# Meryx/ComputeRayTracer

Measured on AMD Instinct MI355X. Metric: Mrays/sec (+ HBM GB/s vs peak), 1080p 250k-tri scene, 1/2/4/8 MI355X, higher is better.
Workload: dtype f32; 1 GPU; S2 atrium250k: 253952 triangles + cornell walls/light, 1920x1080, 64 spp per step (BASELINE config 3)

## Files before the change

computeraytracer_amd/csrc/crt_shade.h:

```cpp
#pragma once
#include "crt_device.h"
#include "crt_math.h"
#include "../../include/crt.h"

namespace crt {

#define CRT_PI 3.14159265359f
#define CRT_INFINITY 2139095040.0f
constexpr uint32_t kMaxDepthPath = 100;
constexpr uint32_t kGrid = 16;
constexpr uint32_t kDiffuse = 0, kLight = 1, kGlass = 2;

struct Rng { uint32_t x, y, z, w; };

__device__ __forceinline__ uint32_t tea(uint32_t v0, uint32_t v1)
{
    uint32_t s0 = 0;
#pragma unroll
    for (int n = 0; n < 16; n++) {
        s0 += 0x9e3779b9u;
        v0 += ((v1 << 4) + 0xa341316cu) ^ (v1 + s0) ^ ((v1 >> 5) + 0xc8013ea4u);
        v1 += ((v0 << 4) + 0xad90777du) ^ (v0 + s0) ^ ((v0 >> 5) + 0x7e95761eu);
    }
    return v0;
// ... 5 lines not shown
    s.y = s.y * 1664525u + 1013904223u;
    s.z = s.z * 1664525u + 1013904223u;
    s.w = s.w * 1664525u + 1013904223u;
    s.x += s.y * s.w; s.y += s.z * s.x; s.z += s.x * s.y; s.w += s.y * s.z;
    s.x ^= s.x >> 16; s.y ^= s.y >> 16; s.z ^= s.z >> 16; s.w ^= s.w >> 16;
    s.x += s.y * s.w; s.y += s.z * s.x; s.z += s.x * s.y; s.w += s.y * s.z;
    return (float)(s.x & 0x00ffffffu) * 5.9604644775390625e-08f;
}

__device__ __forceinline__ f3 xyz(float4 v) { return f3{v.x, v.y, v.z}; }

template <bool LITERAL>
__device__ __forceinline__ bool beats(float t, float t_min, float t_max, uint32_t index,
                                      uint32_t b_index, uint32_t b_slot)
{
    if (LITERAL) return !(t < t_min || t > t_max);
    return (t >= t_min) && (t < t_max || (t == t_max && (b_slot == kNoHit || index > b_index)));
}

template <bool LITERAL>
__device__ __forceinline__ bool hit_test_rec(const float4 A, const float4 B, const float4 C, const float4 D, float hit_pad,
                                             uint32_t slot, f3 o, f3 d, uint32_t exclude, float t_min, float &t_max,
                                             uint32_t &b_index, uint32_t &b_slot)
{
    const uint32_t index = f_bits(B.w);
    if (exclude == index) return false;
    const uint32_t cat = f_bits(A.w) & 3u;
    float t;
    if (cat == 2u) {
        f3 v0 = xyz(A), e1 = xyz(B), e2 = xyz(C);
        f3 pvec = cross(d, e2);
        float det = dot(e1, pvec);
        if (det == 0.0f) return false;
        float inv = 1.0f / det;
        f3 tvec = o - v0;
        float u = dot(tvec, pvec) * inv;
        if (!(u >= 0.0f && u <= 1.0f)) return false;
        f3 qvec = cross(tvec, e1);
        float v = dot(d, qvec) * inv;
        if (!(v >= 0.0f && (u + v) <= 1.0f)) return false;
        t = dot(e2, qvec) * inv;
        if (LITERAL) { if (!(t >= t_min && t <= t_max)) return false; }
        else if (!beats<false>(t, t_min, t_max, index, b_index, b_slot)) return false;
        f3 p = ray_at(o, d, t);
        f3 v1 = v0 + e1, v2 = v0 + e2;
        float pad = hit_pad;
        bool in = p.x >= min_(v0.x, min_(v1.x, v2.x)) - pad && p.x <= max_(v0.x, max_(v1.x, v2.x)) + pad &&
                  p.y >= min_(v0.y, min_(v1.y, v2.y)) - pad && p.y <= max_(v0.y, max_(v1.y, v2.y)) + pad &&
                  p.z >= min_(v0.z, min_(v1.z, v2.z)) - pad && p.z <= max_(v0.z, max_(v1.z, v2.z)) + pad;
        if (!in) return false;
    } else if (cat == 0u) {
        f3 n = xyz(D);
        float ndotd = dot(n, d);
        if (ndotd > 0.0f) { n = -n; ndotd = -ndotd; }
        if (abs_(ndotd) < 0.0001f) return false;
        f3 P0 = xyz(A);
        t = dot(n, P0 - o) / ndotd;
        if (!beats<LITERAL>(t, t_min, t_max, index, b_index, b_slot)) return false;
        f3 m = ray_at(o, d, t) - P0;
        float u = dot(m, xyz(B)) / D.w;
        float v = dot(m, xyz(C)) / C.w;
        if (u < 0.0f || u > 1.0f || v < 0.0f || v > 1.0f) return false;
    } else {
        f3 co = o - xyz(A);
        float a = dot(d, d);
        float b = 2.0f * dot(d, co);
        float c = dot(co, co) - B.y;
        float disc = b * b - 4.0f * a * c;
        if (disc <= 0.0f) return false;
        float sq = sqrt_(disc);
        t = (-b - sq) / (2.0f * a);
        if (LITERAL) {
            if (t < t_min || t > t_max) {
                t = (-b + sq) / (2.0f * a);
                if (t < t_min || t > t_max) return false;
            }
        } else {
            if (t < t_min) t = (-b + sq) / (2.0f * a);
            if (!beats<false>(t, t_min, t_max, index, b_index, b_slot)) return false;
        }
    }
    t_max = t; b_index = index; b_slot = slot;
    return true;
}

template <bool LITERAL>
__device__ __forceinline__ bool hit_test(const DevScene &S, uint32_t slot, f3 o, f3 d, uint32_t exclude,
                                         float t_min, float &t_max, uint32_t &b_index, uint32_t &b_slot)
{
    const float4 A = S.prim[3 * slot + 0];
    const float4 B = S.prim[3 * slot + 1];
    const float4 C = S.prim[3 * slot + 2];
    float4 D = float4{0.0f, 0.0f, 0.0f, 0.0f};
    if (exclude != f_bits(B.w) && (f_bits(A.w) & 3u) == 0u) D = S.primD[slot];
    return hit_test_rec<LITERAL>(A, B, C, D, S.hit_pad, slot, o, d, exclude, t_min, t_max, b_index, b_slot);
}

__device__ __forceinline__ void hit_attributes_rec(const float4 A, const float4 B, const float4 C, const float4 D, f3 o, f3 d,
                                                   float t, f3 &pos, f3 &nrm, uint32_t &meta)
{
    meta = f_bits(A.w);
    const uint32_t cat = meta & 3u;
    pos = ray_at(o, d, t);
    if (cat == 1u) {
        nrm = normalize(pos - xyz(A));
    } else {
        f3 n;
        if (cat == 0u) n = xyz(D);
        else n = normalize(cross(xyz(B), xyz(C)));
        nrm = (dot(n, d) > 0.0f) ? -n : n;
    }
}

__device__ __forceinline__ void hit_attributes(const DevScene &S, uint32_t slot, f3 o, f3 d, float t,
                                               f3 &pos, f3 &nrm, uint32_t &meta)
{
    const float4 A = S.prim[3 * slot + 0];
    const uint32_t cat = f_bits(A.w) & 3u;
    float4 B = float4{0.0f, 0.0f, 0.0f, 0.0f}, C = B, D = B;
    if (cat == 0u) D = S.primD[slot];
    else if (cat == 2u) { B = S.prim[3 * slot + 1]; C = S.prim[3 * slot + 2]; }
    hit_attributes_rec(A, B, C, D, o, d, t, pos, nrm, meta);
}

__device__ __noinline__ void intersect_all(const DevScene &S, f3 o, f3 d, uint32_t exclude, float &t_max,
                                           uint32_t &b_index, uint32_t &b_slot, uint32_t &c_prims)
{
    for (uint32_t i = 0; i < S.nprim; i++)
        hit_test<true>(S, S.slot_of_index[i], o, d, exclude, 0.001f, t_max, b_index, b_slot);
    c_prims += S.nprim;
}

__device__ __forceinline__ bool finite3(f3 v)
{
    return abs_(v.x) < 3.0e38f && abs_(v.y) < 3.0e38f && abs_(v.z) < 3.0e38f;
}

template <bool COUNT>
__device__ __forceinline__ void traverse(const DevScene &S, int *stk, f3 o, f3 d, uint32_t exclude,
                                         bool anyhit, float &t_max, uint32_t &b_index, uint32_t &b_slot,
                                         uint32_t &c_nodes, uint32_t &c_prims)
{
    const float t_min = 0.001f;
    if (S.nprim == 0u) return;
    const float tiny = 1.0e-20f;
    f3 id;
    id.x = 1.0f / (abs_(d.x) > tiny ? d.x : __builtin_copysignf(tiny, d.x));
    id.y = 1.0f / (abs_(d.y) > tiny ? d.y : __builtin_copysignf(tiny, d.y));
    id.z = 1.0f / (abs_(d.z) > tiny ? d.z : __builtin_copysignf(tiny, d.z));
    const f3 oid = f3{o.x * id.x, o.y * id.y, o.z * id.z};
    const uint32_t b_slot_in = b_slot;
    int sp = 0;
    int node = S.root;
    for (;;) {
        if (node >= 0) {
            const float4 *np = S.nodes + 4 * (size_t)node;
            const float4 n0 = np[0], n1 = np[1], n2 = np[2], n3 = np[3];
            float ax = fma_(n0.x, id.x, -oid.x), bx = fma_(n0.w, id.x, -oid.x);
            float ay = fma_(n0.y, id.y, -oid.y), by = fma_(n1.x, id.y, -oid.y);
            float az = fma_(n0.z, id.z, -oid.z), bz = fma_(n1.y, id.z, -oid.z);
            float tn0 = __builtin_fmaxf(__builtin_fmaxf(__builtin_fminf(ax, bx), __builtin_fminf(ay, by)),
                                        __builtin_fmaxf(__builtin_fminf(az, bz), t_min));
            float tf0 = __builtin_fminf(__builtin_fminf(__builtin_fmaxf(ax, bx), __builtin_fmaxf(ay, by)),
                                        __builtin_fminf(__builtin_fmaxf(az, bz), t_max));
            ax = fma_(n1.z, id.x, -oid.x); bx = fma_(n2.y, id.x, -oid.x);
            ay = fma_(n1.w, id.y, -oid.y); by = fma_(n2.z, id.y, -oid.y);
// ... 284 lines not shown
```

computeraytracer_amd/csrc/crt_wavefront.hip:

```cpp
#include "crt_shade.h"
#include "crt_tile_class.h"
#include "crt_launch.h"
#include <algorithm>

namespace crt {

#ifndef CRT_WF_STACK
#define CRT_WF_STACK 32
#endif
#ifndef CRT_WF_REFILL
#define CRT_WF_REFILL 24
#endif
#ifndef CRT_WF_INNER_RUN
#define CRT_WF_INNER_RUN 6
#endif
#ifndef CRT_WF_BURSTS
#define CRT_WF_BURSTS 4
#endif
#ifndef CRT_WF_BVH4
#define CRT_WF_BVH4 1
#endif
#ifndef CRT_WF_LEAF_AT
#define CRT_WF_LEAF_AT 32
#endif
// ... 1239 lines not shown
                        if (k2 < 3.0e38f) { if (sp < kWfStack) stk[sp * 64] = r2; else ovf[(size_t)(sp - kWfStack) * ovl] = r2; sp++; }
                        if (k1 < 3.0e38f) { if (sp < kWfStack) stk[sp * 64] = r1; else ovf[(size_t)(sp - kWfStack) * ovl] = r1; sp++; }
                        if (COUNT) d_max_sp = max(d_max_sp, (uint32_t)sp);
                        node = r0;
                    } else if (sp > 0) {
                        sp--; node = stack_pop(stk, ovf, ovl, sp);
                    } else {
                        node = kNoNode;
                        if (pend == 0) {
                            if (shadow) stnt(&g_vis[slot], (b_slot == b_slot_in) ? 1u : 0u);
                            else stnt(&g_hit[slot], float2{t_max, bits_f(b_slot)});
                            active = false;
                        }
                    }
#else
                    const float4 *np = nodes + 4 * (size_t)node;
                    const float4 n0 = np[0], n1 = np[1], n2 = np[2], n3 = np[3];
                    float ax = fma_(n0.x, id.x, -oid.x), bx = fma_(n0.w, id.x, -oid.x);
                    float ay = fma_(n0.y, id.y, -oid.y), by = fma_(n1.x, id.y, -oid.y);
                    float az = fma_(n0.z, id.z, -oid.z), bz = fma_(n1.y, id.z, -oid.z);
                    float tn0 = __builtin_fmaxf(__builtin_fmaxf(__builtin_fminf(ax, bx), __builtin_fminf(ay, by)),
                                                __builtin_fmaxf(__builtin_fminf(az, bz), t_min));
                    float tf0 = __builtin_fminf(__builtin_fminf(__builtin_fmaxf(ax, bx), __builtin_fmaxf(ay, by)),
                                                __builtin_fminf(__builtin_fmaxf(az, bz), t_max));
                    ax = fma_(n1.z, id.x, -oid.x); bx = fma_(n2.y, id.x, -oid.x);
                    ay = fma_(n1.w, id.y, -oid.y); by = fma_(n2.z, id.y, -oid.y);
                    az = fma_(n2.x, id.z, -oid.z); bz = fma_(n2.w, id.z, -oid.z);
                    float tn1 = __builtin_fmaxf(__builtin_fmaxf(__builtin_fminf(ax, bx), __builtin_fminf(ay, by)),
                                                __builtin_fmaxf(__builtin_fminf(az, bz), t_min));
                    float tf1 = __builtin_fminf(__builtin_fminf(__builtin_fmaxf(ax, bx), __builtin_fmaxf(ay, by)),
                                                __builtin_fminf(__builtin_fmaxf(az, bz), t_max));
                    if (COUNT) c_nodes += 2;
                    const bool h0 = tn0 <= tf0 * 1.0000005f;
                    const bool h1 = tn1 <= tf1 * 1.0000005f;
                    const int r0 = (int)f_bits(n3.x), r1 = (int)f_bits(n3.y);
                    const bool first0 = tn0 <= tn1;
                    if (h0 & h1) {
                        stk[sp * 64] = first0 ? r1 : r0;
                        sp++;
                        node = first0 ? r0 : r1;
                    } else if (h0 | h1) {
                        node = h0 ? r0 : r1;
                    } else if (sp > 0) {
                        sp--; node = stk[sp * 64];
                    } else {
                        node = kNoNode;
                        if (pend == 0) {
                            if (shadow) stnt(&g_vis[slot], (b_slot == b_slot_in) ? 1u : 0u);
                            else stnt(&g_hit[slot], float2{t_max, bits_f(b_slot)});
                            active = false;
                        }
                    }
#endif
                }
            }
        }
    }
    if (COUNT) {
        wave_add(ctl->counters[blockIdx.x % kWfShards] + CRT_CNT_NODES, c_nodes);
        wave_add(ctl->counters[blockIdx.x % kWfShards] + CRT_CNT_PRIMS, c_prims);
        if (lane == 0) {
            atomicAdd(ctl->counters[blockIdx.x % kWfShards] + 8, (unsigned long long)d_inner_it); atomicAdd(ctl->counters[blockIdx.x % kWfShards] + 9, (unsigned long long)d_inner_act);
            atomicAdd(ctl->counters[blockIdx.x % kWfShards] + 10, (unsigned long long)d_leaf_it); atomicAdd(ctl->counters[blockIdx.x % kWfShards] + 11, (unsigned long long)d_leaf_act);
            atomicAdd(ctl->counters[blockIdx.x % kWfShards] + 12, (unsigned long long)d_prim_it); atomicAdd(ctl->counters[blockIdx.x % kWfShards] + 13, (unsigned long long)d_scans); atomicAdd(ctl->counters[blockIdx.x % kWfShards] + 14, (unsigned long long)d_refill);
            atomicAdd(ctl->counters[blockIdx.x % kWfShards] + 15, (unsigned long long)d_refill_lanes);
        }
        for (int off = 32; off > 0; off >>= 1) d_max_sp = max(d_max_sp, (uint32_t)__shfl_xor((int)d_max_sp, off, 64));
        if (lane == 0) atomicMax(&ctl->max_sp[blockIdx.x % kWfShards], d_max_sp);
    }
}

#ifndef CRT_WF_PICK_AT
#define CRT_WF_PICK_AT 8
#endif
#ifndef CRT_WF_PKFMA
#define CRT_WF_PKFMA 0
#endif
#ifndef CRT_WF_LEAF2_AT
#define CRT_WF_LEAF2_AT 28
#endif
#ifndef CRT_WF_STALL_AT
#define CRT_WF_STALL_AT 16
#endif
constexpr int kStk2 = kWfStackLds2;
#ifndef CRT_WF_RING
#define CRT_WF_RING 32
#endif
constexpr uint32_t kRing2 = CRT_WF_RING;

__device__ __forceinline__ int stack_pop2(const int *stk, const int *ovf, size_t ovl, int sp)
{
    int v = stk[(sp < kStk2 ? sp : kStk2 - 1) * 64];
    if (sp >= kStk2) v = *(const volatile int *)(ovf + (size_t)(sp - kStk2) * ovl);
    return v;
}
__device__ __forceinline__ uint32_t mbcnt64(unsigned long long m)
{
    return __builtin_amdgcn_mbcnt_hi((uint32_t)(m >> 32), __builtin_amdgcn_mbcnt_lo((uint32_t)m, 0u));
}
__device__ __forceinline__ unsigned long long hit_key(float t, uint32_t index)
{
    return ((unsigned long long)f_bits(t) << 32) | (unsigned long long)(index == kNoHit ? 0xFFFFFFFFu : 0xFFFFFFFEu - index);
}

#ifndef CRT_WF_T2_WAVES
#define CRT_WF_T2_WAVES 5
#endif
template <bool COUNT>
__global__ __launch_bounds__(64, CRT_WF_T2_WAVES) void k_wf_trace2(const WfParams P, uint32_t it)
{
    __shared__ int lds_stack[kStk2 * 64];
    __shared__ float4 ring[4][kRing2];
    __shared__ uint2 ring_l[kRing2];
    __shared__ unsigned long long cell[64];
    __shared__ uint32_t cslot[64];
    __shared__ uint2 tasks[64];
    WfCtl *ctl = P.ctl;
    const uint4 *__restrict__ nodesq = P.sc.nodes4q;
    const f3 qscale = f3{P.sc.qscale[0], P.sc.qscale[1], P.sc.qscale[2]}, qbase = f3{P.sc.qbase[0], P.sc.qbase[1], P.sc.qbase[2]};
    const float4 *__restrict__ prim = P.sc.prim;
    const float4 *__restrict__ primD = P.sc.primD;
    uint32_t *__restrict__ g_vis = P.vis;
    float2 *__restrict__ g_hit = P.hit;
    const size_t cls_stride = (size_t)P.list_cap * kWfShards;
    const float4 *__restrict__ recA = P.recA + (size_t)((it & 1u) * 4u) * cls_stride;
    const float4 *__restrict__ recB = P.recB + (size_t)((it & 1u) * 4u) * cls_stride;
    const uint4 *__restrict__ recC = P.recC + (size_t)((it & 1u) * 4u) * cls_stride;
    const float hit_pad = P.sc.hit_pad;
    const int root = P.sc.root4;
    int *__restrict__ ovf = P.stack_overflow + ((size_t)blockIdx.x * 64 + lane_id());
    const size_t ovl = P.overflow_lanes;
    const uint32_t nprim = P.sc.nprim;
    const bool fetchD = ((unsigned long long)P.sc.npatch << CRT_WF_PATCH_RECOMPUTE) > (unsigned long long)nprim;
    DevScene S = P.sc;
    S.prim = prim; S.primD = primD;

    const uint32_t ringi = it & 3u;
    const uint32_t lane = lane_id();
    int *stk = lds_stack + lane;
    const float t_min = 0.001f;

    const uint32_t home = wf_home_shard(P);
    uint32_t cur_shard = home, sh_e0 = 0, sh_e1 = 0, sh_e2 = 0, sh_total = 0;
    uint32_t chunk_pos = 0, chunk_end = 0, ring_head = 0, ring_n = 0;
    bool have_shard = false, exhausted = false;
    {
        const WfShard &so = ctl->shard[ringi][cur_shard];
        sh_e0 = so.n[0]; sh_e1 = sh_e0 + so.n[1]; sh_e2 = sh_e1 + so.n[2]; sh_total = sh_e2 + so.n[3];
        have_shard = sh_total > 0u;
    }
    bool active = false;
    int pend = 0;
    f3 o = f3{0, 0, 0}, d = f3{0, 0, 0}, id = f3{0, 0, 0}, oid = f3{0, 0, 0};
    uint32_t excl = 0, slot = 0, b_index = kNoHit, b_slot = kNoHit, b_slot_in = kNoHit;
    float t_max = 0.0f;
    bool shadow = false;
    int node = kNoNode, sp = 0;
    bool gx = false, gy = false, gz = false;
    uint32_t c_nodes = 0, c_prims = 0;
    uint32_t d_inner_it = 0, d_inner_act = 0, d_leaf_it = 0, d_leaf_act = 0, d_prim_it = 0, d_refill = 0, d_refill_lanes = 0, d_scans = 0;
    uint32_t d_max_sp = 0;

    for (;;) {
        const unsigned long long idle = __ballot(!active);
        const int nidle = __popcll(idle);
        if (nidle >= CRT_WF_PICK_AT) {
            if (ring_n == 0u && !exhausted) {
                for (int guard = 0; chunk_pos == chunk_end && !exhausted && guard < 2 * (int)kWfShards; guard++) {
                    if (have_shard) {
                        uint32_t base = 0;
                        if (lane == 0) base = atomicAdd(&ctl->shard[ringi][cur_shard].cur, (uint32_t)kTraceChunk);
                        base = __shfl(base, 0, 64);
                        if (base < sh_total) { chunk_pos = base; chunk_end = min(base + (uint32_t)kTraceChunk, sh_total); break; }
                        have_shard = false;
                    }
                    if (COUNT) d_scans++;
                    const WfShard &sl = ctl->shard[ringi][lane % kWfShards];
                    const uint32_t e0 = sl.n[0], e1 = e0 + sl.n[1], e2 = e1 + sl.n[2], tot = e2 + sl.n[3];
                    const uint32_t cur_l = __hip_atomic_load(&sl.cur, __ATOMIC_RELAXED, __HIP_MEMORY_SCOPE_AGENT);
                    const unsigned long long avail = __ballot(cur_l < tot);
                    if (!avail) { exhausted = true; break; }
                    const uint32_t rot = cur_shard & 63u;
                    const unsigned long long pick = wf_prefer_home(P, avail, home);
                    const unsigned long long rmask = rot ? ((pick >> rot) | (pick << (64u - rot))) : pick;
                    cur_shard = ((uint32_t)(__ffsll((long long)rmask) - 1) + rot) & 63u;
                    sh_e0 = __shfl(e0, (int)cur_shard, 64); sh_e1 = __shfl(e1, (int)cur_shard, 64);
                    sh_e2 = __shfl(e2, (int)cur_shard, 64); sh_total = __shfl(tot, (int)cur_shard, 64);
                    have_shard = true;
                }
                if (chunk_pos < chunk_end) {
                    const uint32_t n = min(kRing2, chunk_end - chunk_pos);
                    bool ok = false;
                    float4 R0 = float4{0, 0, 0, 0}, R1 = R0, R2 = R0, R3 = R0;
                    uint2 RL = uint2{kNoHit, kNoHit};
                    if (lane < n) {
                        const uint32_t idx = chunk_pos + lane;
                        const size_t region = (size_t)cur_shard * P.list_cap;
                        const bool sh = idx >= sh_e1;
                        const size_t g = idx < sh_e0 ? region + idx : idx < sh_e1 ? cls_stride + region + (idx - sh_e0)
                                       : idx < sh_e2 ? 2u * cls_stride + region + (idx - sh_e1) : 3u * cls_stride + region + (idx - sh_e2);
                        const float4 ro = ldnt(&recA[g]), rd = ldnt(&recB[g]);
                        uint4 rc = uint4{0, 0, 0, 0};
                        if (sh) rc = ldnt(&recC[g]);
                        uint32_t r_slot;
                        float r_tmax;
                        ok = true;
                        if (sh) {
                            r_slot = rc.x & kWfListSlot; r_tmax = rd.w;
                            RL = uint2{rc.y, rc.z};
                        } else {
                            r_slot = f_bits(rd.w) & kWfListSlot; r_tmax = CRT_INFINITY;
                            if (f_bits(rd.w) & kWfListAlsoExt) ok = false;
                            else if (nprim == 0u) { g_hit[r_slot] = float2{r_tmax, bits_f(kNoHit)}; ok = false; }
                        }
                        const float tiny = 1.0e-20f;
                        f3 i3;
                        i3.x = 1.0f / (abs_(rd.x) > tiny ? rd.x : __builtin_copysignf(tiny, rd.x));
                        i3.y = 1.0f / (abs_(rd.y) > tiny ? rd.y : __builtin_copysignf(tiny, rd.y));
                        i3.z = 1.0f / (abs_(rd.z) > tiny ? rd.z : __builtin_copysignf(tiny, rd.z));
                        const f3 oi = f3{fma_(qbase.x, i3.x, -(ro.x * i3.x)), fma_(qbase.y, i3.y, -(ro.y * i3.y)), fma_(qbase.z, i3.z, -(ro.z * i3.z))};
                        R0 = ro;
                        R1 = float4{rd.x, rd.y, rd.z, bits_f(r_slot | (sh ? 0x80000000u : 0u))};
                        R2 = float4{qscale.x * i3.x, qscale.y * i3.y, qscale.z * i3.z, r_tmax};
                        R3 = float4{oi.x, oi.y, oi.z, bits_f((i3.x < 0.0f ? 1u : 0u) | (i3.y < 0.0f ? 2u : 0u) | (i3.z < 0.0f ? 4u : 0u))};
                    }
                    const unsigned long long mk = __ballot(ok);
                    if (ok) {
                        const uint32_t e = mbcnt64(mk);
                        ring[0][e] = R0; ring[1][e] = R1; ring[2][e] = R2; ring[3][e] = R3; ring_l[e] = RL;
                    }
                    ring_head = 0; ring_n = (uint32_t)__popcll(mk);
                    chunk_pos += n;
                    if (COUNT) { d_refill++; d_refill_lanes += ring_n; }
                    __builtin_amdgcn_fence(__ATOMIC_RELEASE, "wavefront");
                    __builtin_amdgcn_wave_barrier();
                }
            }
            if (ring_n > 0u) {
                const uint32_t give = min((uint32_t)nidle, ring_n);
                const uint32_t my = mbcnt64(idle);
                if (!active && my < give) {
                    const uint32_t e = ring_head + my;
                    const float4 R0 = ring[0][e], R1 = ring[1][e], R2 = ring[2][e], R3 = ring[3][e];
                    const uint2 RL = ring_l[e];
                    o = xyz(R0); excl = f_bits(R0.w);
                    d = xyz(R1); slot = f_bits(R1.w) & kWfListSlot; shadow = (f_bits(R1.w) >> 31) != 0u;
                    id = xyz(R2); t_max = R2.w;
                    oid = xyz(R3);
                    const uint32_t sg = f_bits(R3.w);
                    gx = (sg & 1u) != 0u; gy = (sg & 2u) != 0u; gz = (sg & 4u) != 0u;
                    b_index = RL.x; b_slot = RL.y; b_slot_in = b_slot;
                    cell[lane] = hit_key(t_max, b_index); cslot[lane] = b_slot;
                    node = root; sp = 0; pend = 0;
                    active = true;
                }
                ring_head += give; ring_n -= give;
            }
        }
        if (__ballot(active) == 0ull) {
            if (exhausted && ring_n == 0u) break;
            continue;
        }

#pragma unroll 1
        for (int pass = 0; pass < 64; pass++) {
            if (active && node < 0 && pend == 0 && sp > 0) {
                pend = node;
                sp--; node = stack_pop2(stk, ovf, ovl, sp);
            }
            const bool inner = active && node >= 0 && node != kNoNode;
            const bool leaf = active && (node < 0 || pend != 0);
            const int ni = __popcll(__ballot(inner)), nl = __popcll(__ballot(leaf)), nb = __popcll(__ballot(active));
            if (nb == 0) break;
            if (pass > 0 && 64 - nb >= CRT_WF_PICK_AT && (ring_n > 0u || !exhausted)) break;
            if (nl >= CRT_WF_LEAF2_AT || ni == 0 || nb - ni >= CRT_WF_STALL_AT) {
                const int lf = pend != 0 ? pend : node;
                const uint32_t cnt = leaf ? ((~(uint32_t)lf) & 7u) + 1u : 0u;
                const unsigned long long c0 = __ballot((cnt & 1u) != 0u), c1 = __ballot((cnt & 2u) != 0u), c2 = __ballot((cnt & 4u) != 0u), c3 = __ballot((cnt & 8u) != 0u);
                const uint32_t pre = mbcnt64(c0) + 2u * mbcnt64(c1) + 4u * mbcnt64(c2) + 8u * mbcnt64(c3);
                const bool incl = leaf && pre + cnt <= 64u;
                const unsigned long long mi = __ballot(incl);
                const uint32_t T = (uint32_t)(__popcll(c0 & mi) + 2 * __popcll(c1 & mi) + 4 * __popcll(c2 & mi) + 8 * __popcll(c3 & mi));
                const uint32_t first = (~(uint32_t)lf) >> 3;
                if (incl) {
                    tasks[pre] = uint2{first, lane};
                    if (cnt > 1u) tasks[pre + 1u] = uint2{first + 1u, lane};
                    if (cnt > 2u) tasks[pre + 2u] = uint2{first + 2u, lane};
                    if (cnt > 3u) tasks[pre + 3u] = uint2{first + 3u, lane};
                    for (uint32_t i = 4; i < cnt; i++) tasks[pre + i] = uint2{first + i, lane};
                }
                __builtin_amdgcn_fence(__ATOMIC_RELEASE, "wavefront");
                __builtin_amdgcn_wave_barrier();
                if (COUNT) { d_leaf_it++; d_leaf_act += T; d_prim_it += 1u; }
                const uint2 tk = lane < T ? tasks[lane] : uint2{0u, lane};
                const int owner = (int)tk.y;
                const uint32_t ps = tk.x;
                float4 A = float4{0, 0, 0, 0}, B = A, C = A, D = A;
                if (lane < T) { A = prim[3 * (size_t)ps + 0]; B = prim[3 * (size_t)ps + 1]; C = prim[3 * (size_t)ps + 2]; if (fetchD) D = primD[ps]; }
                bool from_pend = false;
                if (incl) {
                    from_pend = pend != 0;
                    if (from_pend) pend = 0;
                    else if (sp > 0) { sp--; node = stack_pop2(stk, ovf, ovl, sp); }
                    else node = kNoNode;
                }
                const f3 to = f3{__shfl(o.x, owner, 64), __shfl(o.y, owner, 64), __shfl(o.z, owner, 64)};
                const f3 td = f3{__shfl(d.x, owner, 64), __shfl(d.y, owner, 64), __shfl(d.z, owner, 64)};
                const uint32_t t_excl = (uint32_t)__shfl((int)excl, owner, 64);
                bool acc = false;
                unsigned long long key = 0;
                if (lane < T) {
                    const unsigned long long cur = cell[owner];
                    float tm = bits_f((uint32_t)(cur >> 32));
                    const uint32_t low = (uint32_t)cur;
                    uint32_t bi = low == 0xFFFFFFFFu ? kNoHit : 0xFFFFFFFEu - low;
                    const uint32_t bs0 = low == 0xFFFFFFFFu ? kNoHit : 0xFFFFFFFEu;
                    uint32_t bs = bs0;
                    if ((f_bits(A.w) & 3u) == 2u) tri_test(A, B, C, ps, to, td, t_excl, t_min, hit_pad, tm, bi, bs);
                    else {
                        if (!fetchD && (f_bits(A.w) & 3u) == 0u) { const f3 nn = normalize(cross(xyz(B), xyz(C))); D = float4{nn.x, nn.y, nn.z, dot(xyz(B), xyz(B))}; }
                        hit_test_rec<false>(A, B, C, D, hit_pad, ps, to, td, t_excl, t_min, tm, bi, bs);
                    }
                    if (COUNT && __ballot((f_bits(A.w) & 3u) != 2u) != 0ull) d_scans += 64u;
                    acc = bs != bs0;
                    if (acc) {
                        key = hit_key(tm, bi);
                        atomicMin(&cell[owner], key);
                    }
                    if (COUNT) c_prims++;
                }
                __builtin_amdgcn_fence(__ATOMIC_ACQ_REL, "wavefront");
                __builtin_amdgcn_wave_barrier();
                if (acc && cell[owner] == key) cslot[owner] = ps;
                __builtin_amdgcn_fence(__ATOMIC_ACQ_REL, "wavefront");
                __builtin_amdgcn_wave_barrier();
                if (incl) {
                    const unsigned long long v = cell[lane];
                    const uint32_t low = (uint32_t)v;
                    t_max = bits_f((uint32_t)(v >> 32));
                    b_index = low == 0xFFFFFFFFu ? kNoHit : 0xFFFFFFFEu - low;
                    b_slot = cslot[lane];
                    bool done = false;
                    if (shadow && b_slot != b_slot_in) done = true;
                    else if (node == kNoNode && pend == 0) done = true;
                    if (done) {
                        if (shadow) stnt(&g_vis[slot], (b_slot == b_slot_in) ? 1u : 0u);
                        else stnt(&g_hit[slot], float2{t_max, bits_f(b_slot)});
                        active = false;
                    }
                }
            } else {
                if (COUNT) { d_inner_it++; d_inner_act += (uint32_t)ni; }
                if (inner) {
                    float k0, k1, k2, k3;
                    int r0, r1, r2, r3;
                    const uint4 *nq = (const uint4 *)((const char *)nodesq + ((uint32_t)node << 6));
                    const uint4 Q0 = nq[0], Q1 = nq[1], Q2 = nq[2], Q3 = nq[3];
                    const uint32_t nxa = gx ? Q1.z : Q0.x, nxb = gx ? Q1.w : Q0.y, fxa = gx ? Q0.x : Q1.z, fxb = gx ? Q0.y : Q1.w;
                    const uint32_t nya = gy ? Q2.x : Q0.z, nyb = gy ? Q2.y : Q0.w, fya = gy ? Q0.z : Q2.x, fyb = gy ? Q0.w : Q2.y;
                    const uint32_t nza = gz ? Q2.z : Q1.x, nzb = gz ? Q2.w : Q1.y, fza = gz ? Q1.x : Q2.z, fzb = gz ? Q1.y : Q2.w;
#if CRT_WF_PKFMA
                    {
                        const v2f ix = v2f{id.x, id.x}, iy = v2f{id.y, id.y}, iz = v2f{id.z, id.z};
                        const v2f ox = v2f{oid.x, oid.x}, oy = v2f{oid.y, oid.y}, oz = v2f{oid.z, oid.z};
#define CRT_PK(Q, I, O) __builtin_elementwise_fma(v2f{(float)((Q) & 0xFFFFu), (float)((Q) >> 16)}, I, O)
                        const v2f tnx_a = CRT_PK(nxa, ix, ox), tnx_b = CRT_PK(nxb, ix, ox), tfx_a = CRT_PK(fxa, ix, ox), tfx_b = CRT_PK(fxb, ix, ox);
                        const v2f tny_a = CRT_PK(nya, iy, oy), tny_b = CRT_PK(nyb, iy, oy), tfy_a = CRT_PK(fya, iy, oy), tfy_b = CRT_PK(fyb, iy, oy);
                        const v2f tnz_a = CRT_PK(nza, iz, oz), tnz_b = CRT_PK(nzb, iz, oz), tfz_a = CRT_PK(fza, iz, oz), tfz_b = CRT_PK(fzb, iz, oz);
#undef CRT_PK
#define CRT_QK(K, NX, NY, NZ, FX, FY, FZ) { \
                            const float tn_ = __builtin_fmaxf(__builtin_fmaxf(NX, NY), __builtin_fmaxf(NZ, t_min)); \
                            const float tf_ = __builtin_fminf(__builtin_fminf(FX, FY), __builtin_fminf(FZ, t_max)); \
                            K = (tn_ <= tf_ * 1.0000005f) ? tn_ : 3.0e38f; }
                        CRT_QK(k0, tnx_a.x, tny_a.x, tnz_a.x, tfx_a.x, tfy_a.x, tfz_a.x)
                        CRT_QK(k1, tnx_a.y, tny_a.y, tnz_a.y, tfx_a.y, tfy_a.y, tfz_a.y)
                        CRT_QK(k2, tnx_b.x, tny_b.x, tnz_b.x, tfx_b.x, tfy_b.x, tfz_b.x)
                        CRT_QK(k3, tnx_b.y, tny_b.y, tnz_b.y, tfx_b.y, tfy_b.y, tfz_b.y)
#undef CRT_QK
                    }
#else
#define CRT_QBOX(K, NXQ, NYQ, NZQ, FXQ, FYQ, FZQ) { \
                        const float tn_ = __builtin_fmaxf(__builtin_fmaxf(fma_((float)(NXQ), id.x, oid.x), fma_((float)(NYQ), id.y, oid.y)), \
                                                          __builtin_fmaxf(fma_((float)(NZQ), id.z, oid.z), t_min)); \
                        const float tf_ = __builtin_fminf(__builtin_fminf(fma_((float)(FXQ), id.x, oid.x), fma_((float)(FYQ), id.y, oid.y)), \
                                                          __builtin_fminf(fma_((float)(FZQ), id.z, oid.z), t_max)); \
                        K = (tn_ <= tf_ * 1.0000005f) ? tn_ : 3.0e38f; }
                    CRT_QBOX(k0, nxa & 0xFFFFu, nya & 0xFFFFu, nza & 0xFFFFu, fxa & 0xFFFFu, fya & 0xFFFFu, fza & 0xFFFFu)
                    CRT_QBOX(k1, nxa >> 16, nya >> 16, nza >> 16, fxa >> 16, fya >> 16, fza >> 16)
                    CRT_QBOX(k2, nxb & 0xFFFFu, nyb & 0xFFFFu, nzb & 0xFFFFu, fxb & 0xFFFFu, fyb & 0xFFFFu, fzb & 0xFFFFu)
                    CRT_QBOX(k3, nxb >> 16, nyb >> 16, nzb >> 16, fxb >> 16, fyb >> 16, fzb >> 16)
#undef CRT_QBOX
#endif
                    r0 = (int)Q3.x; r1 = (int)Q3.y; r2 = (int)Q3.z; r3 = (int)Q3.w;
                    if (COUNT) c_nodes += 4;
#define CRT_CAS(ka, ra, kb, rb) { const bool sw_ = kb < ka; const float tk_ = sw_ ? kb : ka; kb = sw_ ? ka : kb; ka = tk_; \
                                  const int tr_ = sw_ ? rb : ra; rb = sw_ ? ra : rb; ra = tr_; }
                    CRT_CAS(k0, r0, k1, r1) CRT_CAS(k2, r2, k3, r3) CRT_CAS(k0, r0, k2, r2) CRT_CAS(k1, r1, k3, r3) CRT_CAS(k1, r1, k2, r2)
#undef CRT_CAS
                    if (k0 < 3.0e38f) {
                        if (k3 < 3.0e38f) { if (sp < kStk2) stk[sp * 64] = r3; else ovf[(size_t)(sp - kStk2) * ovl] = r3; sp++; }
                        if (k2 < 3.0e38f) { if (sp < kStk2) stk[sp * 64] = r2; else ovf[(size_t)(sp - kStk2) * ovl] = r2; sp++; }
                        if (k1 < 3.0e38f) { if (sp < kStk2) stk[sp * 64] = r1; else ovf[(size_t)(sp - kStk2) * ovl] = r1; sp++; }
                        if (COUNT) d_max_sp = max(d_max_sp, (uint32_t)sp);
                        node = r0;
                    } else if (sp > 0) {
                        sp--; node = stack_pop2(stk, ovf, ovl, sp);
                    } else {
                        node = kNoNode;
                        if (pend == 0) {
                            if (shadow) stnt(&g_vis[slot], (b_slot == b_slot_in) ? 1u : 0u);
                            else stnt(&g_hit[slot], float2{t_max, bits_f(b_slot)});
                            active = false;
                        }
                    }
                }
            }
        }
    }
    if (COUNT) {
        wave_add(ctl->counters[blockIdx.x % kWfShards] + CRT_CNT_NODES, c_nodes);
        wave_add(ctl->counters[blockIdx.x % kWfShards] + CRT_CNT_PRIMS, c_prims);
        if (lane == 0) {
            atomicAdd(ctl->counters[blockIdx.x % kWfShards] + 8, (unsigned long long)d_inner_it); atomicAdd(ctl->counters[blockIdx.x % kWfShards] + 9, (unsigned long long)d_inner_act);
            atomicAdd(ctl->counters[blockIdx.x % kWfShards] + 10, (unsigned long long)d_leaf_it); atomicAdd(ctl->counters[blockIdx.x % kWfShards] + 11, (unsigned long long)d_leaf_act);
            atomicAdd(ctl->counters[blockIdx.x % kWfShards] + 12, (unsigned long long)d_prim_it); atomicAdd(ctl->counters[blockIdx.x % kWfShards] + 13, (unsigned long long)d_scans); atomicAdd(ctl->counters[blockIdx.x % kWfShards] + 14, (unsigned long long)d_refill);
            atomicAdd(ctl->counters[blockIdx.x % kWfShards] + 15, (unsigned long long)d_refill_lanes);
        }
        for (int off = 32; off > 0; off >>= 1) d_max_sp = max(d_max_sp, (uint32_t)__shfl_xor((int)d_max_sp, off, 64));
        if (lane == 0) atomicMax(&ctl->max_sp[blockIdx.x % kWfShards], d_max_sp);
    }
}

template <bool COUNT>
__global__ __launch_bounds__(64) void k_wf_finish(const WfParams P, const WfFinishSegs G)
{
    __shared__ int lds_stack[kStackDepth * 64];
    const DevScene &S = P.sc;
    const uint32_t seg = blockIdx.x / G.blocks_per_seg, blk = blockIdx.x % G.blocks_per_seg;
    WfCtl *ctl = G.ctl[seg];
    int *stk = lds_stack + lane_id();
    const uint32_t j = blk * P.tail_bound + threadIdx.x;
    const uint32_t count = min(ctl->side_count[G.batch[seg]], kWfSideCap);
    if (blk == 0 && threadIdx.x == 0 && count > G.blocks_per_seg * P.tail_bound) atomicAdd(&ctl->dropped, count - G.blocks_per_seg * P.tail_bound);
    const bool mine = threadIdx.x < P.tail_bound && j < count;
    const uint32_t slot = G.base[seg] + (mine ? j : 0u);
    uint32_t flags = 0;
    if (mine) flags = P.misc[slot].y;
    bool alive = mine && (flags & kWfAlive);
    bool pend_sh = false, pend_ext = false;
    const bool wide = finish_walks_wide(S);
    ShadeCnt cn;
    uint32_t c_nodes = 0, c_prims = 0;
    for (int guard = 0; guard < 512 && __ballot(alive) != 0ull; guard++) {
        if (alive) {
            const float4 ro = P.ray_o[slot];
            const f3 o = xyz(ro);
            const uint32_t excl = f_bits(ro.w);
            if (pend_sh) {
                const float4 sd = P.sh_d[slot];
                uint32_t how;
                P.vis[slot] = finish_walk_shadow<COUNT>(S, stk, wide, o, xyz(sd), excl, sd.w, P.vis[slot], c_nodes, c_prims, how) ? 1u : 0u;
            }
            if (pend_ext) {
                const float4 rd = P.ray_d[slot];
                if (f_bits(rd.w) == 0u) {
                    float t_max = CRT_INFINITY;
                    uint32_t b_index = kNoHit, b_slot = kNoHit, how;
                    finish_walk_extension<COUNT>(S, stk, wide, o, xyz(rd), excl, t_max, b_index, b_slot, c_nodes, c_prims, how);
                    P.hit[slot] = float2{t_max, bits_f(b_slot)};
                }
            }
            ShadeOut so = shade_body<COUNT, true>(P, slot, true, cn);
            const uint32_t resolved = shade_store<COUNT, true>(P, slot, true, so, cn);
            (void)resolved;
            alive = so.alive; pend_ext = so.emit_ext; pend_sh = so.emit_sh;
        }
    }
    if (alive) atomicAdd(&ctl->dropped, 1u);

    if (COUNT) {
        wave_add(ctl->counters[blockIdx.x % kWfShards] + CRT_CNT_RAYS, cn.rays);
        wave_add(ctl->counters[blockIdx.x % kWfShards] + CRT_CNT_BOUNCES, cn.bounces);
        wave_add(ctl->counters[blockIdx.x % kWfShards] + CRT_CNT_SHADOW, cn.shadow);
        wave_add(ctl->counters[blockIdx.x % kWfShards] + CRT_CNT_HITS, cn.hits);
        wave_add(ctl->counters[blockIdx.x % kWfShards] + CRT_CNT_PATHS, cn.paths);
        wave_add(ctl->counters[blockIdx.x % kWfShards] + CRT_CNT_PRIMS, cn.prims + c_prims);
        wave_add(ctl->counters[blockIdx.x % kWfShards] + CRT_CNT_WALKED, cn.walk);
        wave_add(ctl->counters[blockIdx.x % kWfShards] + CRT_CNT_NODES, c_nodes);
    }
}

__global__ __launch_bounds__(64) void k_wf_resolve(const WfParams P, uint32_t last_sample)
{
    const size_t npix = (size_t)P.tw * P.th;
    const size_t pix = (size_t)blockIdx.x * 64 + threadIdx.x;
// ... 228 lines not shown
```

Before: 8049 Mrays/s.

## Run two inner-node steps per wave iteration when most lanes are inner

Adds an optional double-step of BVH4 inner-node traversal when at least 40 lanes are on inner nodes, so a second node visit happens before returning to the leaf/refill decision loop. Before the second step, a lane holding a leaf with no pending work parks that leaf and pops the next stack entry. Also adds gated-off variants: branch-free flat triangle/patch acceptance tests, and resolving hit slot late from index to drop the cslot LDS array and a barrier. Only the double-step is on by default. It trades extra divergence and longer per-iteration latency for fewer scheduling round trips.

```diff
diff --git a/computeraytracer_amd/csrc/crt_shade.h b/computeraytracer_amd/csrc/crt_shade.h
--- a/computeraytracer_amd/csrc/crt_shade.h
+++ b/computeraytracer_amd/csrc/crt_shade.h
@@ -111,6 +111,52 @@
     }
     t_max = t; b_index = index; b_slot = slot;
     return true;
+}
+
+__device__ __forceinline__ bool beats_flat(float t, float t_min, float t_max, uint32_t index, uint32_t b_index, uint32_t b_slot)
+{
+    return (t >= t_min) & ((t < t_max) | ((t == t_max) & ((b_slot == kNoHit) | (index > b_index))));
+}
+
+__device__ __forceinline__ bool tri_accepts_flat(const float4 A, const float4 B, const float4 C, float hit_pad, f3 o, f3 d,
+                                                 uint32_t exclude, float t_min, float t_max, uint32_t b_index, uint32_t b_slot, float &t)
+{
+    const uint32_t index = f_bits(B.w);
+    const f3 v0 = xyz(A), e1 = xyz(B), e2 = xyz(C);
+    const f3 pvec = cross(d, e2);
+    const float det = dot(e1, pvec);
+    const float inv = 1.0f / det;
+    const f3 tvec = o - v0;
+    const float u = dot(tvec, pvec) * inv;
+    const f3 qvec = cross(tvec, e1);
+    const float v = dot(d, qvec) * inv;
+    t = dot(e2, qvec) * inv;
+    const f3 p = ray_at(o, d, t);
+    const f3 v1 = v0 + e1, v2 = v0 + e2;
+    const f3 lo = f3{min_(v0.x, min_(v1.x, v2.x)) - hit_pad, min_(v0.y, min_(v1.y, v2.y)) - hit_pad, min_(v0.z, min_(v1.z, v2.z)) - hit_pad};
+    const f3 hi = f3{max_(v0.x, max_(v1.x, v2.x)) + hit_pad, max_(v0.y, max_(v1.y, v2.y)) + hit_pad, max_(v0.z, max_(v1.z, v2.z)) + hit_pad};
+    const bool in = (p.x >= lo.x) & (p.x <= hi.x) & (p.y >= lo.y) & (p.y <= hi.y) & (p.z >= lo.z) & (p.z <= hi.z);
+    const bool wins = beats_flat(t, t_min, t_max, index, b_index, b_slot);
+    return (exclude != index) & (det != 0.0f) & (u >= 0.0f) & (u <= 1.0f) & (v >= 0.0f) & ((u + v) <= 1.0f) & wins & in;
+}
+
+__device__ __forceinline__ bool patch_accepts_flat(const float4 A, const float4 B, const float4 C, const float4 D, f3 o, f3 d,
+                                                   uint32_t exclude, float t_min, float t_max, uint32_t b_index, uint32_t b_slot, float &t)
+{
+    const uint32_t index = f_bits(B.w);
+    f3 n = xyz(D);
+    float ndotd = dot(n, d);
+    const bool flip = ndotd > 0.0f;
+    n = f3{flip ? -n.x : n.x, flip ? -n.y : n.y, flip ? -n.z : n.z};
+    ndotd = flip ? -ndotd : ndotd;
+    const f3 P0 = xyz(A);
+    t = dot(n, P0 - o) / ndotd;
+    const f3 m = ray_at(o, d, t) - P0;
+    const float u = dot(m, xyz(B)) / D.w;
+    const float v = dot(m, xyz(C)) / C.w;
+    const bool grazing = abs_(ndotd) < 0.0001f;
+    const bool wins = beats_flat(t, t_min, t_max, index, b_index, b_slot);
+    return (exclude != index) & !grazing & wins & !((u < 0.0f) | (u > 1.0f) | (v < 0.0f) | (v > 1.0f));
 }
 
 template <bool LITERAL>
diff --git a/computeraytracer_amd/csrc/crt_wavefront.hip b/computeraytracer_amd/csrc/crt_wavefront.hip
--- a/computeraytracer_amd/csrc/crt_wavefront.hip
+++ b/computeraytracer_amd/csrc/crt_wavefront.hip
@@ -1345,6 +1345,21 @@
 #ifndef CRT_WF_STALL_AT
 #define CRT_WF_STALL_AT 16
 #endif
+#ifndef CRT_WF_T2_DOUBLE
+#define CRT_WF_T2_DOUBLE 1
+#endif
+#ifndef CRT_WF_T2_DOUBLE_AT
+#define CRT_WF_T2_DOUBLE_AT 40
+#endif
+#ifndef CRT_WF_T2_FLAT
+#define CRT_WF_T2_FLAT 0
+#endif
+#ifndef CRT_WF_T2_LATE_SLOT
+#define CRT_WF_T2_LATE_SLOT 0
+#endif
+#if defined(CRT_WF_T2_SETUP64) && CRT_WF_T2_SETUP64
+#error "CRT_WF_T2_SETUP64 was not built (DESIGN.md 5.12): the ring set-up stays at 32 lanes"
+#endif
 constexpr int kStk2 = kWfStackLds2;
 #ifndef CRT_WF_RING
 #define CRT_WF_RING 32
@@ -1376,7 +1391,9 @@
     __shared__ float4 ring[4][kRing2];
     __shared__ uint2 ring_l[kRing2];
     __shared__ unsigned long long cell[64];
+#if !CRT_WF_T2_LATE_SLOT
     __shared__ uint32_t cslot[64];
+#endif
     __shared__ uint2 tasks[64];
     WfCtl *ctl = P.ctl;
     const uint4 *__restrict__ nodesq = P.sc.nodes4q;
@@ -1415,7 +1432,11 @@
     bool active = false;
     int pend = 0;
     f3 o = f3{0, 0, 0}, d = f3{0, 0, 0}, id = f3{0, 0, 0}, oid = f3{0, 0, 0};
-    uint32_t excl = 0, slot = 0, b_index = kNoHit, b_slot = kNoHit, b_slot_in = kNoHit;
+    uint32_t excl = 0, slot = 0, b_index = kNoHit;
+    uint32_t b_in = kNoHit;
+#if !CRT_WF_T2_LATE_SLOT
+    uint32_t b_slot = kNoHit;
+#endif
     float t_max = 0.0f;
     bool shadow = false;
     int node = kNoNode, sp = 0;
@@ -1423,6 +1444,15 @@
     uint32_t c_nodes = 0, c_prims = 0;
     uint32_t d_inner_it = 0, d_inner_act = 0, d_leaf_it = 0, d_leaf_act = 0, d_prim_it = 0, d_refill = 0, d_refill_lanes = 0, d_scans = 0;
     uint32_t d_max_sp = 0;
+    auto ray_out = [&]() {
+#if CRT_WF_T2_LATE_SLOT
+        if (shadow) stnt(&g_vis[slot], (b_index == b_in) ? 1u : 0u);
+        else stnt(&g_hit[slot], float2{t_max, bits_f(b_index == kNoHit ? kNoHit : P.sc.slot_of_index[b_index])});
+#else
+        if (shadow) stnt(&g_vis[slot], (b_slot == b_in) ? 1u : 0u);
+        else stnt(&g_hit[slot], float2{t_max, bits_f(b_slot)});
+#endif
+    };
 
     for (;;) {
         const unsigned long long idle = __ballot(!active);
@@ -1512,8 +1542,14 @@
                     oid = xyz(R3);
                     const uint32_t sg = f_bits(R3.w);
                     gx = (sg & 1u) != 0u; gy = (sg & 2u) != 0u; gz = (sg & 4u) != 0u;
-                    b_index = RL.x; b_slot = RL.y; b_slot_in = b_slot;
+                    b_index = RL.x;
+#if CRT_WF_T2_LATE_SLOT
+                    b_in = b_index;
+                    cell[lane] = hit_key(t_max, b_index);
+#else
+                    b_slot = RL.y; b_in = b_slot;
                     cell[lane] = hit_key(t_max, b_index); cslot[lane] = b_slot;
+#endif
                     node = root; sp = 0; pend = 0;
                     active = true;
                 }
@@ -1579,11 +1615,27 @@
                     uint32_t bi = low == 0xFFFFFFFFu ? kNoHit : 0xFFFFFFFEu - low;
                     const uint32_t bs0 = low == 0xFFFFFFFFu ? kNoHit : 0xFFFFFFFEu;
                     uint32_t bs = bs0;
+#if CRT_WF_T2_FLAT
+                    const uint32_t cat = f_bits(A.w) & 3u;
+                    bool ok;
+                    float t = tm;
+                    if (!fetchD && cat == 0u) { const f3 nn = normalize(cross(xyz(B), xyz(C))); D = float4{nn.x, nn.y, nn.z, dot(xyz(B), xyz(B))}; }
+                    if (cat == 2u) {
+                        ok = tri_accepts_flat(A, B, C, hit_pad, to, td, t_excl, t_min, tm, bi, bs, t);
+                    } else if (cat == 0u && CRT_WF_T2_FLAT != 2) {
+                        ok = patch_accepts_flat(A, B, C, D, to, td, t_excl, t_min, tm, bi, bs, t);
+                    } else {
+                        uint32_t si = bi, ss = bs;
+                        ok = hit_test_rec<false>(A, B, C, D, hit_pad, ps, to, td, t_excl, t_min, t, si, ss);
+                    }
+                    tm = ok ? t : tm; bi = ok ? f_bits(B.w) : bi; bs = ok ? ps : bs;
+#else
                     if ((f_bits(A.w) & 3u) == 2u) tri_test(A, B, C, ps, to, td, t_excl, t_min, hit_pad, tm, bi, bs);
                     else {
                         if (!fetchD && (f_bits(A.w) & 3u) == 0u) { const f3 nn = normalize(cross(xyz(B), xyz(C))); D = float4{nn.x, nn.y, nn.z, dot(xyz(B), xyz(B))}; }
                         hit_test_rec<false>(A, B, C, D, hit_pad, ps, to, td, t_excl, t_min, tm, bi, bs);
                     }
+#endif
                     if (COUNT && __ballot((f_bits(A.w) & 3u) != 2u) != 0ull) d_scans += 64u;
                     acc = bs != bs0;
                     if (acc) {
@@ -1594,86 +1646,101 @@
                 }
                 __builtin_amdgcn_fence(__ATOMIC_ACQ_REL, "wavefront");
                 __builtin_amdgcn_wave_barrier();
+#if !CRT_WF_T2_LATE_SLOT
                 if (acc && cell[owner] == key) cslot[owner] = ps;
                 __builtin_amdgcn_fence(__ATOMIC_ACQ_REL, "wavefront");
                 __builtin_amdgcn_wave_barrier();
+#endif
                 if (incl) {
                     const unsigned long long v = cell[lane];
                     const uint32_t low = (uint32_t)v;
                     t_max = bits_f((uint32_t)(v >> 32));
                     b_index = low == 0xFFFFFFFFu ? kNoHit : 0xFFFFFFFEu - low;
+#if CRT_WF_T2_LATE_SLOT
+                    const bool beaten = b_index != b_in;
+#else
                     b_slot = cslot[lane];
+                    const bool beaten = b_slot != b_in;
+#endif
                     bool done = false;
-                    if (shadow && b_slot != b_slot_in) done = true;
+                    if (shadow && beaten) done = true;
                     else if (node == kNoNode && pend == 0) done = true;
-                    if (done) {
-                        if (shadow) stnt(&g_vis[slot], (b_slot == b_slot_in) ? 1u : 0u);
-                        else stnt(&g_hit[slot], float2{t_max, bits_f(b_slot)});
-                        active = false;
-                    }
+                    if (done) { ray_out(); active = false; }
                 }
             } else {
-                if (COUNT) { d_inner_it++; d_inner_act += (uint32_t)ni; }
-                if (inner) {
-                    float k0, k1, k2, k3;
-                    int r0, r1, r2, r3;
-                    const uint4 *nq = (const uint4 *)((const char *)nodesq + ((uint32_t)node << 6));
-                    const uint4 Q0 = nq[0], Q1 = nq[1], Q2 = nq[2], Q3 = nq[3];
-                    const uint32_t nxa = gx ? Q1.z : Q0.x, nxb = gx ? Q1.w : Q0.y, fxa = gx ? Q0.x : Q1.z, fxb = gx ? Q0.y : Q1.w;
-                    const uint32_t nya = gy ? Q2.x : Q0.z, nyb = gy ? Q2.y : Q0.w, fya = gy ? Q0.z : Q2.x, fyb = gy ? Q0.w : Q2.y;
-                    const uint32_t nza = gz ? Q2.z : Q1.x, nzb = gz ? Q2.w : Q1.y, fza = gz ? Q1.x : Q2.z, fzb = gz ? Q1.y : Q2.w;
+#if CRT_WF_T2_DOUBLE
+                const int steps = ni >= CRT_WF_T2_DOUBLE_AT ? 2 : 1;
+#else
+                const int steps = 1;
+#endif
+                bool on = inner;
+#pragma unroll 1
+                for (int st = 0; st < steps; st++) {
+                    if (st > 0) {
+                        if (active && node < 0 && pend == 0 && sp > 0) {
+                            pend = node;
+                            sp--; node = stack_pop2(stk, ovf, ovl, sp);
+                        }
+                        on = active && node >= 0 && node != kNoNode;
+                    }
+                    if (COUNT) { d_inner_it++; d_inner_act += st > 0 ? (uint32_t)__popcll(__ballot(on)) : (uint32_t)ni; }
+                    if (on) {
+                        float k0, k1, k2, k3;
+                        int r0, r1, r2, r3;
+                        const uint4 *nq = (const uint4 *)((const char *)nodesq + ((uint32_t)node << 6));
+                        const uint4 Q0 = nq[0], Q1 = nq[1], Q2 = nq[2], Q3 = nq[3];
+                        const uint32_t nxa = gx ? Q1.z : Q0.x, nxb = gx ? Q1.w : Q0.y, fxa = gx ? Q0.x : Q1.z, fxb = gx ? Q0.y : Q1.w;
+                        const uint32_t nya = gy ? Q2.x : Q0.z, nyb = gy ? Q2.y : Q0.w, fya = gy ? Q0.z : Q2.x, fyb = gy ? Q0.w : Q2.y;
+                        const uint32_t nza = gz ? Q2.z : Q1.x, nzb = gz ? Q2.w : Q1.y, fza = gz ? Q1.x : Q2.z, fzb = gz ? Q1.y : Q2.w;
 #if CRT_WF_PKFMA
-                    {
-                        const v2f ix = v2f{id.x, id.x}, iy = v2f{id.y, id.y}, iz = v2f{id.z, id.z};
-                        const v2f ox = v2f{oid.x, oid.x}, oy = v2f{oid.y, oid.y}, oz = v2f{oid.z, oid.z};
+                        {
+                            const v2f ix = v2f{id.x, id.x}, iy = v2f{id.y, id.y}, iz = v2f{id.z, id.z};
+                            const v2f ox = v2f{oid.x, oid.x}, oy = v2f{oid.y, oid.y}, oz = v2f{oid.z, oid.z};
 #define CRT_PK(Q, I, O) __builtin_elementwise_fma(v2f{(float)((Q) & 0xFFFFu), (float)((Q) >> 16)}, I, O)
-                        const v2f tnx_a = CRT_PK(nxa, ix, ox), tnx_b = CRT_PK(nxb, ix, ox), tfx_a = CRT_PK(fxa, ix, ox), tfx_b = CRT_PK(fxb, ix, ox);
-                        const v2f tny_a = CRT_PK(nya, iy, oy), tny_b = CRT_PK(nyb, iy, oy), tfy_a = CRT_PK(fya, iy, oy), tfy_b = CRT_PK(fyb, iy, oy);
-                        const v2f tnz_a = CRT_PK(nza, iz, oz), tnz_b = CRT_PK(nzb, iz, oz), tfz_a = CRT_PK(fza, iz, oz), tfz_b = CRT_PK(fzb, iz, oz);
+                            const v2f tnx_a = CRT_PK(nxa, ix, ox), tnx_b = CRT_PK(nxb, ix, ox), tfx_a = CRT_PK(fxa, ix, ox), tfx_b = CRT_PK(fxb, ix, ox);
+                            const v2f tny_a = CRT_PK(nya, iy, oy), tny_b = CRT_PK(nyb, iy, oy), tfy_a = CRT_PK(fya, iy, oy), tfy_b = CRT_PK(fyb, iy, oy);
+                            const v2f tnz_a = CRT_PK(nza, iz, oz), tnz_b = CRT_PK(nzb, iz, oz), tfz_a = CRT_PK(fza, iz, oz), tfz_b = CRT_PK(fzb, iz, oz);
 #undef CRT_PK
 #define CRT_QK(K, NX, NY, NZ, FX, FY, FZ) { \
-                            const float tn_ = __builtin_fmaxf(__builtin_fmaxf(NX, NY), __builtin_fmaxf(NZ, t_min)); \
-                            const float tf_ = __builtin_fminf(__builtin_fminf(FX, FY), __builtin_fminf(FZ, t_max)); \
-                            K = (tn_ <= tf_ * 1.0000005f) ? tn_ : 3.0e38f; }
-                        CRT_QK(k0, tnx_a.x, tny_a.x, tnz_a.x, tfx_a.x, tfy_a.x, tfz_a.x)
-                        CRT_QK(k1, tnx_a.y, tny_a.y, tnz_a.y, tfx_a.y, tfy_a.y, tfz_a.y)
-                        CRT_QK(k2, tnx_b.x, tny_b.x, tnz_b.x, tfx_b.x, tfy_b.x, tfz_b.x)
-                        CRT_QK(k3, tnx_b.y, tny_b.y, tnz_b.y, tfx_b.y, tfy_b.y, tfz_b.y)
+                                const float tn_ = __builtin_fmaxf(__builtin_fmaxf(NX, NY), __builtin_fmaxf(NZ, t_min)); \
+                                const float tf_ = __builtin_fminf(__builtin_fminf(FX, FY), __builtin_fminf(FZ, t_max)); \
+                                K = (tn_ <= tf_ * 1.0000005f) ? tn_ : 3.0e38f; }
+                            CRT_QK(k0, tnx_a.x, tny_a.x, tnz_a.x, tfx_a.x, tfy_a.x, tfz_a.x)
+                            CRT_QK(k1, tnx_a.y, tny_a.y, tnz_a.y, tfx_a.y, tfy_a.y, tfz_a.y)
+                            CRT_QK(k2, tnx_b.x, tny_b.x, tnz_b.x, tfx_b.x, tfy_b.x, tfz_b.x)
+                            CRT_QK(k3, tnx_b.y, tny_b.y, tnz_b.y, tfx_b.y, tfy_b.y, tfz_b.y)
 #undef CRT_QK
-                    }
+                        }
 #else
 #define CRT_QBOX(K, NXQ, NYQ, NZQ, FXQ, FYQ, FZQ) { \
-                        const float tn_ = __builtin_fmaxf(__builtin_fmaxf(fma_((float)(NXQ), id.x, oid.x), fma_((float)(NYQ), id.y, oid.y)), \
-                                                          __builtin_fmaxf(fma_((float)(NZQ), id.z, oid.z), t_min)); \
-                        const float tf_ = __builtin_fminf(__builtin_fminf(fma_((float)(FXQ), id.x, oid.x), fma_((float)(FYQ), id.y, oid.y)), \
-                                                          __builtin_fminf(fma_((float)(FZQ), id.z, oid.z), t_max)); \
-                        K = (tn_ <= tf_ * 1.0000005f) ? tn_ : 3.0e38f; }
-                    CRT_QBOX(k0, nxa & 0xFFFFu, nya & 0xFFFFu, nza & 0xFFFFu, fxa & 0xFFFFu, fya & 0xFFFFu, fza & 0xFFFFu)
-                    CRT_QBOX(k1, nxa >> 16, nya >> 16, nza >> 16, fxa >> 16, fya >> 16, fza >> 16)
-                    CRT_QBOX(k2, nxb & 0xFFFFu, nyb & 0xFFFFu, nzb & 0xFFFFu, fxb & 0xFFFFu, fyb & 0xFFFFu, fzb & 0xFFFFu)
-                    CRT_QBOX(k3, nxb >> 16, nyb >> 16, nzb >> 16, fxb >> 16, fyb >> 16, fzb >> 16)
+                            const float tn_ = __builtin_fmaxf(__builtin_fmaxf(fma_((float)(NXQ), id.x, oid.x), fma_((float)(NYQ), id.y, oid.y)), \
+                                                              __builtin_fmaxf(fma_((float)(NZQ), id.z, oid.z), t_min)); \
+                            const float tf_ = __builtin_fminf(__builtin_fminf(fma_((float)(FXQ), id.x, oid.x), fma_((float)(FYQ), id.y, oid.y)), \
+                                                              __builtin_fminf(fma_((float)(FZQ), id.z, oid.z), t_max)); \
+                            K = (tn_ <= tf_ * 1.0000005f) ? tn_ : 3.0e38f; }
+                        CRT_QBOX(k0, nxa & 0xFFFFu, nya & 0xFFFFu, nza & 0xFFFFu, fxa & 0xFFFFu, fya & 0xFFFFu, fza & 0xFFFFu)
+                        CRT_QBOX(k1, nxa >> 16, nya >> 16, nza >> 16, fxa >> 16, fya >> 16, fza >> 16)
+                        CRT_QBOX(k2, nxb & 0xFFFFu, nyb & 0xFFFFu, nzb & 0xFFFFu, fxb & 0xFFFFu, fyb & 0xFFFFu, fzb & 0xFFFFu)
+                        CRT_QBOX(k3, nxb >> 16, nyb >> 16, nzb >> 16, fxb >> 16, fyb >> 16, fzb >> 16)
 #undef CRT_QBOX
 #endif
-                    r0 = (int)Q3.x; r1 = (int)Q3.y; r2 = (int)Q3.z; r3 = (int)Q3.w;
-                    if (COUNT) c_nodes += 4;
+                        r0 = (int)Q3.x; r1 = (int)Q3.y; r2 = (int)Q3.z; r3 = (int)Q3.w;
+                        if (COUNT) c_nodes += 4;
 #define CRT_CAS(ka, ra, kb, rb) { const bool sw_ = kb < ka; const float tk_ = sw_ ? kb : ka; kb = sw_ ? ka : kb; ka = tk_; \
-                                  const int tr_ = sw_ ? rb : ra; rb = sw_ ? ra : rb; ra = tr_; }
-                    CRT_CAS(k0, r0, k1, r1) CRT_CAS(k2, r2, k3, r3) CRT_CAS(k0, r0, k2, r2) CRT_CAS(k1, r1, k3, r3) CRT_CAS(k1, r1, k2, r2)
+                                      const int tr_ = sw_ ? rb : ra; rb = sw_ ? ra : rb; ra = tr_; }
+                        CRT_CAS(k0, r0, k1, r1) CRT_CAS(k2, r2, k3, r3) CRT_CAS(k0, r0, k2, r2) CRT_CAS(k1, r1, k3, r3) CRT_CAS(k1, r1, k2, r2)
 #undef CRT_CAS
-                    if (k0 < 3.0e38f) {
-                        if (k3 < 3.0e38f) { if (sp < kStk2) stk[sp * 64] = r3; else ovf[(size_t)(sp - kStk2) * ovl] = r3; sp++; }
-                        if (k2 < 3.0e38f) { if (sp < kStk2) stk[sp * 64] = r2; else ovf[(size_t)(sp - kStk2) * ovl] = r2; sp++; }
-                        if (k1 < 3.0e38f) { if (sp < kStk2) stk[sp * 64] = r1; else ovf[(size_t)(sp - kStk2) * ovl] = r1; sp++; }
-                        if (COUNT) d_max_sp = max(d_max_sp, (uint32_t)sp);
-                        node = r0;
-                    } else if (sp > 0) {
-                        sp--; node = stack_pop2(stk, ovf, ovl, sp);
-                    } else {
-                        node = kNoNode;
-                        if (pend == 0) {
-                            if (shadow) stnt(&g_vis[slot], (b_slot == b_slot_in) ? 1u : 0u);
-                            else stnt(&g_hit[slot], float2{t_max, bits_f(b_slot)});
-                            active = false;
+                        if (k0 < 3.0e38f) {
+                            if (k3 < 3.0e38f) { if (sp < kStk2) stk[sp * 64] = r3; else ovf[(size_t)(sp - kStk2) * ovl] = r3; sp++; }
+                            if (k2 < 3.0e38f) { if (sp < kStk2) stk[sp * 64] = r2; else ovf[(size_t)(sp - kStk2) * ovl] = r2; sp++; }
+                            if (k1 < 3.0e38f) { if (sp < kStk2) stk[sp * 64] = r1; else ovf[(size_t)(sp - kStk2) * ovl] = r1; sp++; }
+                            if (COUNT) d_max_sp = max(d_max_sp, (uint32_t)sp);
+                            node = r0;
+                        } else if (sp > 0) {
+                            sp--; node = stack_pop2(stk, ovf, ovl, sp);
+                        } else {
+                            node = kNoNode;
+                            if (pend == 0) { ray_out(); active = false; }
                         }
                     }
                 }
```

Result: faster. 8174 Mrays/s, median of 6 (+1.6%).
